# OpenStitching/stitching

Hardware: AMD Instinct MI355X
Metric: warped+blended Mpix/s (higher is better)
Workload: dtype u8/int16 (fixed-point remap, int32 pyramid sums, fp32 weights); 1 GPU; BASELINE config 2: 8 synthetic 4000x3000 frames, one ring; yaw step 38.9 deg = 0.58 hfov (42 % overlap; SURVEY 8(d) names 0.70 hfov); spherical warp + 5-band multiband blend, inputs resident in HBM; frames_per_gpu=8, panoramas_in_flight=2

## Files before the change

include/stitching_amd_debug.h:

```cpp
#ifndef STITCHING_AMD_DEBUG_H
#define STITCHING_AMD_DEBUG_H

#include "stitching_amd.h"

#ifdef __cplusplus
extern "C" {
#endif

int stx_debug_warp_maps(stx_ctx* ctx, int type, float scale, const float K[9], const float R[9], int w, int h, int which,
                        const int rect_xywh[4], stx_buf** out_xmap_f32, stx_buf** out_ymap_f32, int out_xywh[4]);

int stx_debug_feather_dist_cap(void);

int stx_debug_blend_replayed(stx_ctx* ctx, int* out_launches);

int stx_debug_warp_table_launches(stx_ctx* ctx, int* out_launches);

int stx_debug_blend_uploads(stx_ctx* ctx, int* out_uploads);

int stx_debug_blend_mask_stored(stx_ctx* ctx, int* out_stored);

#ifdef __cplusplus
}
#endif
#endif
```

stitching_amd/_lib.py:

```python
import ctypes as C
import os

from .stitching_error import StitchingError

_HERE = os.path.dirname(os.path.abspath(__file__))
LIB_PATH = os.environ.get("STITCHING_AMD_LIB") or os.path.join(_HERE, "libstitching_amd.so")

STX_OK = 0
WARP_PLANE, WARP_AFFINE, WARP_CYLINDRICAL, WARP_SPHERICAL = 0, 1, 2, 3
WARP_TYPE_IDS = {"plane": 0, "affine": 1, "cylindrical": 2, "spherical": 3, "fisheye": 4, "stereographic": 5,
                 "compressedPlaneA2B1": 6, "compressedPlaneA1.5B1": 7, "compressedPlanePortraitA2B1": 8,
                 "compressedPlanePortraitA1.5B1": 9, "paniniA2B1": 10, "paniniA1.5B1": 11, "paniniPortraitA2B1": 12,
                 "paniniPortraitA1.5B1": 13, "mercator": 14, "transverseMercator": 15}
INTER_NEAREST, INTER_LINEAR = 0, 1
BORDER_CONSTANT, BORDER_REFLECT = 0, 2
BLEND_NO, BLEND_FEATHER, BLEND_MULTIBAND = 0, 1, 2
U8, S16, F32 = 0, 1, 2
TRIG_MODES = {"exact": 0, "glibc": 1, "glibc-nofma": 2}
REMAP_MODES = {"q15": 0, "float": 1, "float-fma": 2}
PYRDOWN_MODES = {"scalar": 0, "simd-v": 1, "simd-hv": 3, "simd-v-fma": 5, "simd-hv-fma": 7}
GAIN_MAP_BOUNDED = 1
EXPOSURE_KINDS = {"gain": 1, "gain_blocks": 2, "channel": 3, "channel_blocks": 4}
EXPOSURE_SOLVERS = {"host": 0, "device": 1}
LU_NB, LU_MAX_N = 32, 16384
# ... 79 lines not shown
    "stx_blend_use_weights": [_vp, _vp, _ip],
    "stx_mb_weights_free": [_vp],
    "stx_blend_set_band": [_vp, _i, _i],
    "stx_blend_feed_ex": [_vp, _vp, _vp, _i, _i, _i],
    "stx_blend_contrib_rect": [_vp, _i, _i, _i, _i, _i, _i, _ip, _zp],
    "stx_blend_export_contrib": [_vp, _i, _i, _i, _vpp, _ip],
    "stx_blend_export_contribs": [_vp, _i, _ip, _ip, _ip, _vpp, _ip],
    "stx_blend_build": [_vp],
    "stx_blend_feed_contrib_ex": [_vp, _i, _ip, _vp, _i],
    "stx_buf_flags": [_vp, _ip],
    "stx_strip_rect": [_vp, _i, _i, _i, _i, _i, _i, _ip, _zp],
    "stx_view_rect": [_vp, _i, _i, _i, _i, _i, _i, _i, _i, _ip],
    "stx_strip_pack": [_vp, _vp, _vp, _i, _i, _vpp],
    "stx_strip_pack_batch_ex": [_vp, _i, _vpp, _vpp, _ip, _ip, _i, _vpp],
    "stx_strip_bytes": [_i, _i, _i, _zp],
    "stx_strip_unpack": [_vp, _i, _i, _i, _vpp, _vpp],
    "stx_blend_feed_strips": [_vp, _i, _vpp, _ip, _ip, _ip, _ip, _ip, _i],
    "stx_comm_unique_id": [_ubp],
    "stx_comm_create": [_vp, _i, _i, _ubp, _vpp],
    "stx_comm_exchange_begin_on": [_vp, _vp, _i, _ip, _ip, _vpp, _zp],
    "stx_comm_exchange_end_on": [_vp, _vp],
    "stx_comm_info": [_vp, _ip],
    "stx_comm_destroy": [_vp],
    "stx_prof_enable": [_vp, _i],
    "stx_prof_reset": [_vp],
    "stx_prof_count": [_vp, _ip],
    "stx_prof_get": [_vp, _i, C.c_char_p, _i, C.POINTER(C.c_int64), _dp, _dp],
    "stx_mark": [_vp, _i],
    "stx_mark_elapsed_ms": [_vp, _i, _i, _dp],
    "stx_exposure_stats": [_vp, _i, _i, _vpp, _vpp, _ip, _i, _llp, _ip, _llp, _dp],
    "stx_exposure_solve": [_i, _i, _ip, _dp, _ubp, _dp],
    "stx_set_exposure_solver": [_i],
    "stx_get_exposure_solver": [],
    "stx_exposure_feed_ex": [_vp, _i, _i, _vpp, _vpp, _ip, _i, _i, _i, _dp, _llp, _dp],
    "stx_exposure_solve_device": [_vp, _i, _i, _ip, _dp, _ubp, _dp, _dp],
    "stx_lu_solve_device": [_vp, _i, _dp, _dp, _dp, _dp],
    "stx_seam_find": [_vp, _i, _i, _ip, _ip, _vpp, _vpp, _dp],
    "stx_seam_schedule": [_i, _ip, _ip, _ip, _ip, _ip],
    "stx_color_seam_find": [_vp, _i, _ip, _ip, _vpp, _vpp, _vpp, _dp],
    "stx_crop_lir": [_vp, _vp, _ip, _ip, _dp],
    "stx_features_detect": [_vp, _i, _vpp, _vpp, _i, _i, _i, _ip, _ip, _ip, _ip, C.POINTER(C.c_byte), _ip, _ip, _llp, _ubp, _dp],
    "stx_match_features": [_vp, _i, _vpp, _ip, _vpp, _ip, _i, _i, _i, _d, _u, _ip, _ip, _ubp, _ip, _dp, _dp],
    "stx_match_features_model": [_vp, _i, _vpp, _ip, _vpp, _ip, _i, _i, _i, _d, _u, _i, _ip, _ip, _ubp, _ip, _dp, _dp],
    "stx_ray_problem_create": [_vp, _i, _ip, _llp, _dp, _vpp],
    "stx_ray_problem_eval": [_vp, _i, _dp, _dp, _dp],
    "stx_affine_problem_eval": [_vp, _i, _dp, _dp, _dp],
    "stx_reproj_problem_eval": [_vp, _i, _dp, _dp, _dp],
    "stx_ray_problem_free": [_vp],
    "stx_ingest": [_vp, _i, C.POINTER(ForeignFrame), _i, _i, _vp, _i, _vpp],
    "stx_emit": [_vp, _i, C.POINTER(EmitItem), _i, _i, _vp, _i, _vpp],
    "stx_debug_warp_maps": [_vp, _i, _f, _fp, _fp, _i, _i, _i, _ip, _vpp, _vpp, _ip],
    "stx_debug_feather_dist_cap": [],
    "stx_debug_blend_replayed": [_vp, _ip],
    "stx_debug_warp_table_launches": [_vp, _ip],
    "stx_debug_blend_uploads": [_vp, _ip],
    "stx_debug_blend_mask_stored": [_vp, _ip],
}
EXPORTS = tuple(PROTOTYPES)

_lib = None


def build_hint():
    return "build it with `make -C stitching_amd/csrc` or `python -c 'import __graft_entry__ as g; g.build()'`"


def lib():
    global _lib
    if _lib is not None:
        return _lib
    if not os.path.exists(LIB_PATH):
        raise ImportError(f"{LIB_PATH} is missing: the HIP back end is not built ({build_hint()}). "
                          "stitching_amd has no CPU fallback.")
    L = C.CDLL(LIB_PATH)
    for name, argtypes in PROTOTYPES.items():
        fn = getattr(L, name)
        fn.argtypes = argtypes
        fn.restype = C.c_char_p if name == "stx_last_error" else C.c_int
    _lib = L
    return L


def check(rc):
    if rc != STX_OK:
        msg = lib().stx_last_error()
        raise StitchingError(f"stitching_amd [{rc}]: {msg.decode(errors='replace') if msg else 'unknown error'}")
```

stitching_amd/csrc/stx_blend_fast.hip:

```cpp
#include <algorithm>
#include <cstdlib>

#include "stx_blend_kernels.h"
#include "stx_device_math.h"

using namespace stxd;

namespace {

constexpr int L0_WAVES = 5;
constexpr float WEIGHT_EPS = 1e-5f;
constexpr float INV255 = 0.0039215688593685627f;
constexpr float INV256 = 0.00390625f;

#define STX_GAS __attribute__((address_space(1)))
template <class T> STX_DEV const STX_GAS T* gp(const T* p) { return (const STX_GAS T*)p; }
template <class T> STX_DEV STX_GAS T* gp(T* p) { return (STX_GAS T*)p; }

STX_DEV bool xcd_tile(const StxTileMap& M, uint32_t b, int& tx, int& ty)
{
    if (M.plain) {
        const uint32_t wy = M.tiles_x == 1 ? b : __umulhi(b, M.magic_tx);
        tx = (int)(b - wy * (uint32_t)M.tiles_x);
        ty = (int)wy;
// ... 166 lines not shown
{
    vm0 = vm1 = 0xffffffffu;
    if (__builtin_amdgcn_ballot_w64(lx0 < 0 || lx0 + 8 > iw) != 0ull) {
        const int lo = max(-lx0, 0), hi = min(iw - lx0, 8);
        const uint32_t bits = ((1u << hi) - 1u) & ~((1u << lo) - 1u);
        vm0 = (((bits & 15u) * 0x00204081u) & 0x01010101u) * 0xffu;
        vm1 = (((bits >> 4) * 0x00204081u) & 0x01010101u) * 0xffu;
    }
}
STX_DEV void load_px8_u8(const uint8_t* img0, uint32_t img0_stride, const uint8_t* mask0, uint32_t mask0_stride, int lx0, int ly, uint32_t vm0,
                         uint32_t vm1, uint32_t (&pw)[6], uint32_t (&mw)[2])
{
    const uint32_t off = (uint32_t)ly * img0_stride + (uint32_t)(lx0 * 3 + 64);
    const STX_GAS uint8_t* q = gp(img0) - 64 + (off & ~3u);
    const uint32_t s = off & 3u;
    const v4u d0 = *reinterpret_cast<const STX_GAS v4u_a4*>(q);
    const v4u d1 = *reinterpret_cast<const STX_GAS v4u_a4*>(q + 16);
    pw[0] = __builtin_amdgcn_alignbyte(d0.y, d0.x, s);
    pw[1] = __builtin_amdgcn_alignbyte(d0.z, d0.y, s);
    pw[2] = __builtin_amdgcn_alignbyte(d0.w, d0.z, s);
    pw[3] = __builtin_amdgcn_alignbyte(d1.x, d0.w, s);
    pw[4] = __builtin_amdgcn_alignbyte(d1.y, d1.x, s);
    pw[5] = __builtin_amdgcn_alignbyte(d1.z, d1.y, s);
    const uint32_t moff = (uint32_t)ly * mask0_stride + (uint32_t)(lx0 + 64);
    const STX_GAS uint8_t* mq = gp(mask0) - 64 + (moff & ~3u);
    const uint32_t ms = moff & 3u;
    const uint32_t m0 = *reinterpret_cast<const STX_GAS uint32_t*>(mq), m1 = *reinterpret_cast<const STX_GAS uint32_t*>(mq + 4),
                   m2 = *reinterpret_cast<const STX_GAS uint32_t*>(mq + 8);
    mw[0] = __builtin_amdgcn_alignbyte(m1, m0, ms) & vm0;
    mw[1] = __builtin_amdgcn_alignbyte(m2, m1, ms) & vm1;
}
STX_DEV void load_px8_u8(const StxMbImage& im, int lx0, int ly, uint32_t vm0, uint32_t vm1, uint32_t (&pw)[6], uint32_t (&mw)[2])
{
    load_px8_u8(im.img0, (uint32_t)im.img0_stride, im.mask0, (uint32_t)im.mask0_stride, lx0, ly, vm0, vm1, pw, mw);
}

STX_DEV int s16lo(uint32_t v) { return (int)(short)(v & 0xffffu); }
STX_DEV int s16hi(uint32_t v) { return (int)(short)(v >> 16); }
STX_DEV uint32_t pack16(int lo, int hi) { return ((uint32_t)lo & 0xffffu) | ((uint32_t)hi << 16); }
STX_DEV uint32_t byte_of(const uint32_t* w, int k) { return (w[k >> 2] >> (8 * (k & 3))) & 255u; }

STX_DEV float h5f(float s0, float s1, float s2, float s3, float s4)
{
    return fadd(fadd(fadd(fmul(s2, 6.f), fmul(fadd(s1, s3), 4.f)), s0), s4);
}
STX_DEV int h5i(int s0, int s1, int s2, int s3, int s4) { return s2 * 6 + (s1 + s3) * 4 + s0 + s4; }

constexpr int DN_TOW = 64, DN_TOH = 14, DN_ROWS = 2 * DN_TOH + 3;
constexpr int DN_BAND = 1;
constexpr int LV_WAVES = 1, LV_TH = 2 * LV_WAVES, LV_THREADS = 64 * LV_WAVES;
constexpr int LV_BAND_ROWS = 8;
constexpr int LV_BAND = LV_BAND_ROWS / LV_TH;

STX_DEV void dn_load36(const STX_GAS uint8_t* img, uint32_t off, uint32_t (&w)[9])
{
    const STX_GAS uint8_t* q = img + (off & ~3u);
    const uint32_t s = off & 3u;
    const v4u d0 = *reinterpret_cast<const STX_GAS v4u_a4*>(q);
    const v4u d1 = *reinterpret_cast<const STX_GAS v4u_a4*>(q + 16);
    const v2u d2 = *reinterpret_cast<const STX_GAS v2u_a4*>(q + 32);
    w[0] = __builtin_amdgcn_alignbyte(d0.y, d0.x, s);
    w[1] = __builtin_amdgcn_alignbyte(d0.z, d0.y, s);
    w[2] = __builtin_amdgcn_alignbyte(d0.w, d0.z, s);
    w[3] = __builtin_amdgcn_alignbyte(d1.x, d0.w, s);
    w[4] = __builtin_amdgcn_alignbyte(d1.y, d1.x, s);
    w[5] = __builtin_amdgcn_alignbyte(d1.z, d1.y, s);
    w[6] = __builtin_amdgcn_alignbyte(d1.w, d1.z, s);
    w[7] = __builtin_amdgcn_alignbyte(d2.x, d1.w, s);
    w[8] = __builtin_amdgcn_alignbyte(d2.y, d2.x, s);
}
template <bool MIRROR, int C>
STX_DEV void dn_pack5_channel(const uint32_t* w, short* hs)
{
#define STX_PXB(k) (MIRROR ? 30 - 3 * (k) + C : 3 * (k) + C)
    const pk16 A = pk(pair_u8<STX_PXB(0), STX_PXB(2)>(w)), Bp = pk(pair_u8<STX_PXB(1), STX_PXB(3)>(w));
    const pk16 Cp = pk(pair_u8<STX_PXB(2), STX_PXB(4)>(w)), D = pk(pair_u8<STX_PXB(3), STX_PXB(5)>(w));
    const pk16 E = pk(pair_u8<STX_PXB(4), STX_PXB(6)>(w)), F = pk(pair_u8<STX_PXB(5), STX_PXB(7)>(w));
    const pk16 G = pk(pair_u8<STX_PXB(6), STX_PXB(8)>(w)), H = pk(pair_u8<STX_PXB(7), STX_PXB(9)>(w));
    const pk16 I = pk(pair_u8<STX_PXB(8), STX_PXB(10)>(w));
#undef STX_PXB
    const pk16 o01 = A + E + Cp * pk_splat(6) + (Bp + D) * pk_splat(4);
    const pk16 o23 = E + I + G * pk_splat(6) + (F + H) * pk_splat(4);
    *reinterpret_cast<uint2*>(hs) = make_uint2(unpk(o01), unpk(o23));
}

STX_DEV float4 dn_mask_sums4(const uint32_t (&mb)[3])
{
    const pk16 o01 = pk(pair_u8<0, 2>(mb)) + pk(pair_u8<4, 6>(mb)) + pk(pair_u8<2, 4>(mb)) * pk_splat(6) +
                     (pk(pair_u8<1, 3>(mb)) + pk(pair_u8<3, 5>(mb))) * pk_splat(4);
    const pk16 o23 = pk(pair_u8<4, 6>(mb)) + pk(pair_u8<8, 10>(mb)) + pk(pair_u8<6, 8>(mb)) * pk_splat(6) +
                     (pk(pair_u8<5, 7>(mb)) + pk(pair_u8<7, 9>(mb))) * pk_splat(4);
    return make_float4((float)(unpk(o01) & 0xffffu), (float)(unpk(o01) >> 16), (float)(unpk(o23) & 0xffffu), (float)(unpk(o23) >> 16));
}

struct DnImage0 {
    int fw, fh, iw, ih, left, top;
    uint32_t img0_stride, mask0_stride;
    const uint8_t* img0;
    const uint8_t* mask0;
};
template <bool PK, bool NEAR, bool WEIGHTS, class IM>
STX_DEV void dn_task_level0(const IM& im, int row, int xo, short* hs0, short* hs1, short* hs2, float* hw)
{
    const int by = reflect101_near(row, im.fh) - im.top;
    const bool yin = (unsigned)by < (unsigned)im.ih;
    const int sy = NEAR ? reflect_near(by, im.ih) : reflect(by, im.ih);
    const STX_GAS uint8_t* img = gp(im.img0);
    const uint32_t rowoff = (uint32_t)sy * (uint32_t)im.img0_stride;
    const int c0 = 2 * xo - 2;
    const int a0 = c0 - im.left;
    int px[11][3];
    float f[11];
    if (c0 >= 0 && c0 + 10 < im.fw && a0 >= 0 && a0 + 10 < im.iw) {
        uint32_t w[9];
        dn_load36(img, rowoff + (uint32_t)a0 * 3u, w);
        dn_pack5_channel<false, 0>(w, hs0);
        dn_pack5_channel<false, 1>(w, hs1);
        dn_pack5_channel<false, 2>(w, hs2);
        if (!WEIGHTS) return;
        uint32_t mw[3] = {0u, 0u, 0u};
        if (yin) {
            const uint32_t moff = (uint32_t)by * (uint32_t)im.mask0_stride + (uint32_t)a0;
            const STX_GAS uint8_t* mq = gp(im.mask0) + (moff & ~3u);
            const uint32_t ms = moff & 3u;
            const v4u m = *reinterpret_cast<const STX_GAS v4u_a4*>(mq);
            mw[0] = __builtin_amdgcn_alignbyte(m.y, m.x, ms);
            mw[1] = __builtin_amdgcn_alignbyte(m.z, m.y, ms);
            mw[2] = __builtin_amdgcn_alignbyte(m.w, m.z, ms) & 0x00ffffffu;
        }
        bool packed = PK;
        if (!PK) {
            const uint32_t odd = (mw[0] ^ (((mw[0] >> 7) & 0x01010101u) * 255u)) | (mw[1] ^ (((mw[1] >> 7) & 0x01010101u) * 255u)) |
                                 (mw[2] ^ (((mw[2] >> 7) & 0x01010101u) * 255u));
            packed = __builtin_amdgcn_ballot_w64(odd != 0u) == 0ull;
        }
// ... 435 lines not shown
            for (int j = 0; j < 19; j++) f[j] = wq[reflect101_near(c0 + j, iw)];
        }
        dn_hsum_store_f(f, &s_w[r][4 * q]);
    }
    __syncthreads();
    const int p = tid & 31, rg = tid >> 5;
    const int xo = X0 + 2 * p;
    if (xo >= ow) return;
    const bool two = xo + 1 < ow;
    uint32_t nz = 0u;
#pragma unroll
    for (int rr = 0; rr < 2; rr++) {
        const int yl = 2 * rg + rr, y = Y0 + yl;
        if (yl >= DN_TOH || y >= oh) break;
#pragma unroll
        for (int c = 0; c < 3; c++) {
            int a[5], b[5];
#pragma unroll
            for (int k = 0; k < 5; k++) {
                a[k] = s_h[c][2 * yl + k][p];
                b[k] = s_h[c][2 * yl + k][32 + p];
            }
            const int va = (h5i(a[0], a[1], a[2], a[3], a[4]) + 128) >> 8;
            const int vb = (h5i(b[0], b[1], b[2], b[3], b[4]) + 128) >> 8;
            const uint32_t oo = (uint32_t)c * gopl + (uint32_t)y * gos + (uint32_t)xo;
            if (g8b) {
                STX_GAS uint8_t* o = gp(reinterpret_cast<uint8_t*>(Go_a)) + oo;
                if (two) *reinterpret_cast<STX_GAS uint16_t*>(o) = (uint16_t)((uint32_t)va | ((uint32_t)vb << 8));
                else o[0] = (uint8_t)va;
            } else {
                STX_GAS short* o = gp(reinterpret_cast<short*>(Go_a)) + oo;
                if (two) *reinterpret_cast<STX_GAS uint32_t*>(o) = pack16(va, vb);
                else o[0] = (short)va;
            }
        }
        if (!WEIGHTS) continue;
        float fa[5], fb[5];
#pragma unroll
        for (int k = 0; k < 5; k++) {
            fa[k] = s_w[2 * yl + k][p];
            fb[k] = s_w[2 * yl + k][32 + p];
        }
        const float wa = fmul(h5f(fa[0], fa[1], fa[2], fa[3], fa[4]), INV256);
        const float wb = fmul(h5f(fb[0], fb[1], fb[2], fb[3], fb[4]), INV256);
        STX_GAS float* o = gp(reinterpret_cast<float*>(Wo_a)) + ((uint32_t)y * wost + (uint32_t)xo);
        typedef float v2fl __attribute__((ext_vector_type(2)));
        if (two) { const v2fl wab = {wa, wb}; *reinterpret_cast<STX_GAS v2fl*>(o) = wab; }
        else o[0] = wa;
        nz |= __float_as_uint(wa) | (two ? __float_as_uint(wb) : 0u);
    }
    if (WEIGHTS) dn_note_occ(occ, nz, tid, X0, Y0, ow, oh);
}

STX_DEV int s6(int v) { return (v + 32) >> 6; }

STX_DEV int trunc_small(float v) { return (int)v; }

template <class T>
STX_DEV void up_patch(const T* __restrict__ plane, long long stride, int cw, int ch, int cx, int cy, int up[2][8])
{
    const int rr[3] = {up_idx(cy - 1, ch), cy, up_idx(cy + 1, ch)};
    const bool le = cx == 0, re = cx + 4 >= cw;
    int he[3][4], ho[3][4];
#pragma unroll
    for (int r = 0; r < 3; r++) {
        const T* p = plane + (long long)rr[r] * stride;
        int c[6];
        if (sizeof(T) == 2) {
            const v4u w = *reinterpret_cast<const v4u_a4*>(p + cx - 2);
            c[1] = s16lo(w.y); c[2] = s16hi(w.y); c[3] = s16lo(w.z); c[4] = s16hi(w.z);
            c[0] = s16hi(w.x);
            c[5] = s16lo(w.w);
        } else {
            const v3u w = *reinterpret_cast<const v3u_a4*>(p + cx - 4);
            c[0] = (int)(w.x >> 24);
            c[1] = (int)(w.y & 255u); c[2] = (int)((w.y >> 8) & 255u); c[3] = (int)((w.y >> 16) & 255u); c[4] = (int)(w.y >> 24);
            c[5] = (int)(w.z & 255u);
        }
        if (le) c[0] = c[2];
        if (re) c[5] = c[4];
#pragma unroll
        for (int j = 0; j < 4; j++) {
            he[r][j] = c[j] + 6 * c[j + 1] + c[j + 2];
            ho[r][j] = 4 * (c[j + 1] + c[j + 2]);
        }
    }
#pragma unroll
    for (int j = 0; j < 4; j++) {
        up[0][2 * j] = s6(he[0][j] + 6 * he[1][j] + he[2][j]);
        up[0][2 * j + 1] = s6(ho[0][j] + 6 * ho[1][j] + ho[2][j]);
        up[1][2 * j] = s6(4 * (he[1][j] + he[2][j]));
        up[1][2 * j + 1] = s6(4 * (ho[1][j] + ho[2][j]));
    }
}

template <bool L0, bool MASK_OPT = false>
STX_DEV void level_epilogue(const MbLevelK& P, int X0, int Y0, int (&acc)[2][8][3], float (&ws)[2][8])
{
    int v[2][8][3];
#pragma unroll
    for (int r = 0; r < 2; r++)
#pragma unroll
        for (int j = 0; j < 8; j++) {
            const float den = fadd(ws[r][j], WEIGHT_EPS);
            float q0, q1, q2;
            div3_shared(den, (float)(short)acc[r][j][0], (float)(short)acc[r][j][1], (float)(short)acc[r][j][2], q0, q1, q2);
// ... 1083 lines not shown
#pragma unroll
        for (int c = 0; c < 3; c++) {
            const short* plane = P.up + c * P.up_plane - ((long long)P.up_y0 * P.up_stride + P.up_x0);
            pk16s up[2][4];
            if (!up_patch_pks_math(uw[c], usel, up)) {
                int u32[2][8];
                up_patch(plane, P.up_stride, P.pw >> 1, P.ph >> 1, X0 >> 1, Y0 >> 1, u32);
#pragma unroll
                for (int r = 0; r < 2; r++) {
                    up[r][0] = pks(pack16(u32[r][0], u32[r][2]));
                    up[r][1] = pks(pack16(u32[r][4], u32[r][6]));
                    up[r][2] = pks(pack16(u32[r][1], u32[r][3]));
                    up[r][3] = pks(pack16(u32[r][5], u32[r][7]));
                }
            }
#pragma unroll
            for (int r = 0; r < 2; r++)
#pragma unroll
                for (int q = 0; q < 4; q++) v[r][c][q] = unpks(__builtin_elementwise_add_sat(up[r][q], pks(v[r][c][q])));
        }
    }
#pragma unroll
    for (int r = 0; r < 2; r++) {
        if (Y0 + r >= P.y1) break;
#pragma unroll
        for (int c = 0; c < 3; c++) {
            v4u o;
            o.x = __builtin_amdgcn_perm(v[r][c][2], v[r][c][0], 0x05040100u);
            o.y = __builtin_amdgcn_perm(v[r][c][2], v[r][c][0], 0x07060302u);
            o.z = __builtin_amdgcn_perm(v[r][c][3], v[r][c][1], 0x05040100u);
            o.w = __builtin_amdgcn_perm(v[r][c][3], v[r][c][1], 0x07060302u);
            *reinterpret_cast<STX_GAS v4u*>(gp(P.out) + c * P.out_plane + (long long)(Y0 + r - P.out_y0) * P.out_stride + (X0 - P.out_x0)) = o;
        }
    }
}

static_assert(LV_WAVES == 1, "a cover word is the search of ONE wavefront: a tile of more wavefronts needs a word per wavefront");
__global__ __launch_bounds__(LV_THREADS) void mb_cover_kernel(const StxMbImage* images, int n_images, int level, int x0, int y0, StxTileMap tiles,
                                                              unsigned long long* cover)
{
    const int tid = threadIdx.x;
    int tile_tx, tile_ty;
    if (!xcd_tile(tiles, blockIdx.x, tile_tx, tile_ty)) return;
    const int tile_x = x0 + tile_tx * 512, tile_y = y0 + tile_ty * LV_TH;
    const int Y0 = tile_y + __builtin_amdgcn_readfirstlane(tid >> 6) * 2;
    const bool hit = level == 0 ? mb_tile_hit<true, false>(images, n_images, 0, tile_x, Y0, tid & 63)
                                : mb_tile_hit<false, false>(images, n_images, level, tile_x, Y0, tid & 63);
    const unsigned long long word = __ballot(hit);
    if ((tid & 63) == 0) cover[((Y0 - y0) / LV_TH) * tiles.tiles_x + tile_tx] = word;
}

bool launched_ok() { return hipGetLastError() == hipSuccess; }

}

bool stx_fast_mb_down_batch(stx_ctx* ctx, const StxMbImage* d_images, const StxMbImage* h_images, int n, int level, bool weights)
{
    int mw = 0, mh = 0;
    for (int i = 0; i < n; i++) {
        mw = std::max(mw, (h_images[i].fw >> level) >> 1);
        mh = std::max(mh, (h_images[i].fh >> level) >> 1);
    }
    if (n <= 0 || mw < 1 || mh < 1 || n > 65535) return false;
    StxTileMap M = stx_tile_map((mw + DN_TOW - 1) / DN_TOW, (mh + DN_TOH - 1) / DN_TOH, DN_BAND);
    constexpr int DN_PLAIN_FROM = 3;
    M.plain = level >= DN_PLAIN_FROM;
    bool pk_ok = true;
    for (int i = 0; i < n; i++) pk_ok = pk_ok && !h_images[i].img0_is_s16 && h_images[i].mask_binary;
    dim3 grid(stx_tile_grid(M), 1, n);
    static const unsigned pad_lds = getenv("STITCHING_AMD_D0_LDS") ? (unsigned)atoi(getenv("STITCHING_AMD_D0_LDS")) : 0u;
    if (!weights) {
        if (level == 0 && pk_ok) hipLaunchKernelGGL((mb_down0_lds_kernel<true, false>), grid, dim3(256), pad_lds, ctx->stream, d_images, M);
        else if (level == 0) hipLaunchKernelGGL((mb_down0_lds_kernel<false, false>), grid, dim3(256), 0, ctx->stream, d_images, M);
        else hipLaunchKernelGGL(mb_down_lds_kernel<false>, grid, dim3(256), 0, ctx->stream, d_images, level, M);
    } else if (level == 0 && pk_ok) hipLaunchKernelGGL((mb_down0_lds_kernel<true, true>), grid, dim3(256), pad_lds, ctx->stream, d_images, M);
    else if (level == 0) hipLaunchKernelGGL((mb_down0_lds_kernel<false, true>), grid, dim3(256), 0, ctx->stream, d_images, M);
    else hipLaunchKernelGGL(mb_down_lds_kernel<true>, grid, dim3(256), 0, ctx->stream, d_images, level, M);
    return launched_ok();
}

static bool fast_level_ok(const MbLevelK& K, MbLevelK* KT)
{
    if (K.num_bands - K.level < 3) return false;
    if ((K.x0 | K.y0 | K.out_x0 | K.out_y0 | K.pano_x0 | K.pano_y0) & 7) return false;
    if (K.up && ((K.up_x0 | K.up_y0) & 3)) return false;
    if (K.n_images > 255) return false;
    *KT = K;
    KT->tiles = stx_tile_map((K.x1 - K.x0 + 511) / 512, (K.y1 - K.y0 + LV_TH - 1) / LV_TH, LV_BAND);
    return true;
}

int stx_fast_mb_emit_class(const MbLevelK& K, MbLevelK* KT)
{
    if (!(K.level > 0 || K.all_u8) || !fast_level_ok(K, KT)) { *KT = K; return -1; }
    return K.level == 0 ? 0 : (K.all_u8 ? 1 : 2);
}

bool stx_fast_mb_emit_launch(stx_ctx* ctx, int cls, const MbLevelK* d_Ks, const MbLevelK* h_Ks, int count)
{
    unsigned gx = 1;
    for (int i = 0; i < count; i++) gx = std::max(gx, stx_tile_grid(h_Ks[i].tiles));
    const dim3 grid(gx, 1, (unsigned)count);
    if (cls == 0) hipLaunchKernelGGL((mb_emit_multi_kernel<true, false>), grid, dim3(LV_THREADS), 0, ctx->stream, d_Ks);
    else if (cls == 1) hipLaunchKernelGGL((mb_emit_multi_kernel<false, true>), grid, dim3(LV_THREADS), 0, ctx->stream, d_Ks);
    else hipLaunchKernelGGL((mb_emit_multi_kernel<false, false>), grid, dim3(LV_THREADS), 0, ctx->stream, d_Ks);
    return launched_ok();
}

static bool no_defer()
{
    static const bool off = getenv("STITCHING_AMD_NO_DEFER") != nullptr;
    return off;
}

static bool mb_replays(const MbLevelK& K) { return !K.emit && K.cover != nullptr && K.n_images <= 64 && !K.has_contrib; }
enum MbL0Path { L0_OTHER, L0_PK, L0_DEFER };
// ... 96 lines not shown
```

stitching_amd/csrc/stx_blend_host.cpp:

```cpp
#include <algorithm>
#include <climits>
#include <cmath>
#include <cstdlib>
#include <cstring>
#include <memory>

#include "stx_blend_kernels.h"
#include "stx_internal.h"

STX_EXPORT int stx_debug_feather_dist_cap(void) { return STX_FEATHER_DIST_CAP; }

STX_EXPORT int stx_result_roi(int n, const int* corners_xy, const int* sizes_wh, int out_xywh[4])
{
    if (n <= 0 || !corners_xy || !sizes_wh || !out_xywh) return stx_fail(STX_ERR_INVALID, "bad argument");
    int tlx = INT_MAX, tly = INT_MAX, brx = INT_MIN, bry = INT_MIN;
    for (int i = 0; i < n; i++) {
        tlx = std::min(tlx, corners_xy[2 * i]);
        tly = std::min(tly, corners_xy[2 * i + 1]);
        brx = std::max(brx, corners_xy[2 * i] + sizes_wh[2 * i]);
        bry = std::max(bry, corners_xy[2 * i + 1] + sizes_wh[2 * i + 1]);
    }
    out_xywh[0] = tlx; out_xywh[1] = tly; out_xywh[2] = brx - tlx; out_xywh[3] = bry - tly;
    return STX_OK;
}
// ... 512 lines not shown

STX_EXPORT int stx_blend_keep_weights(stx_blender* b, stx_mb_weights** out)
{
    if (!b || !out) return stx_fail(STX_ERR_INVALID, "null argument");
    *out = nullptr;
    if (b->finished) return stx_fail(STX_ERR_STATE, "keep_weights after blend()");
    if (b->keep) return stx_fail(STX_ERR_STATE, "keep_weights was already called on this blender");
    if (b->images.empty() || !mb_weights_eligible(b, false)) return STX_OK;
    stx_mb_weights* w = new stx_mb_weights();
    w->ctx = b->ctx;
    w->refs = 2;
    b->keep = w;
    *out = w;
    return STX_OK;
}

STX_EXPORT int stx_blend_use_weights(stx_blender* b, stx_mb_weights* w, int* out_adopted)
{
    if (!b || !w || !out_adopted) return stx_fail(STX_ERR_INVALID, "null argument");
    *out_adopted = 0;
    if (b->finished) return stx_fail(STX_ERR_STATE, "use_weights after blend()");
    if (b->ctx != w->ctx) return stx_fail(STX_ERR_INVALID, "use_weights: the handle belongs to another context (no cross-stream use)");
    if (b->adopted || b->keep || w->images.empty() || w->images.size() != b->images.size() || !mb_weights_eligible(b, false)) return STX_OK;
    if (b->num_bands != w->num_bands || b->pyr_mode != w->pyr_mode || b->rx != w->rx || b->ry != w->ry || b->rw != w->rw || b->rh != w->rh)
        return STX_OK;
    for (size_t i = 0; i < b->images.size(); i++) {
        const StxMbImage& im = b->images[i];
        const StxMbKept& k = w->images[i];
        if (b->built[i]) return STX_OK;
        if (im.mask0 != k.mask0 || im.mask0_stride != k.mask0_stride || im.mask_binary != k.mask_binary || im.w1_f16 != k.w1_f16 ||
            im.iw != k.iw || im.ih != k.ih || im.ix != k.ix || im.iy != k.iy || im.fx != k.fx || im.fy != k.fy || im.fw != k.fw ||
            im.fh != k.fh || im.left != k.left || im.top != k.top)
            return STX_OK;
        for (int l = 1; l <= b->num_bands; l++)
            if (im.wt_stride[l] != k.wt_stride[l]) return STX_OK;
    }
    STX_TRY(stx_set_device(b->ctx));
    for (size_t i = 0; i < b->images.size(); i++)
        for (int l = 1; l <= b->num_bands; l++) { b->images[i].wt[l] = w->images[i].wt[l]; b->images[i].occ[l] = w->images[i].occ[l]; }
    b->d_all = nullptr;
    w->refs++;
    b->adopted = w;
    *out_adopted = 1;
    return STX_OK;
}

STX_EXPORT int stx_debug_blend_replayed(stx_ctx* ctx, int* out_launches)
{
    if (!ctx || !out_launches) return stx_fail(STX_ERR_INVALID, "null argument");
    *out_launches = ctx->blend_replayed;
    return STX_OK;
}

STX_EXPORT int stx_debug_blend_mask_stored(stx_ctx* ctx, int* out_stored)
{
    if (!ctx || !out_stored) return stx_fail(STX_ERR_INVALID, "null argument");
    *out_stored = ctx->blend_mask_stored;
    return STX_OK;
}

STX_EXPORT int stx_debug_blend_uploads(stx_ctx* ctx, int* out_uploads)
{
    if (!ctx || !out_uploads) return stx_fail(STX_ERR_INVALID, "null argument");
    *out_uploads = ctx->blend_uploads;
    return STX_OK;
}

STX_EXPORT int stx_mb_weights_free(stx_mb_weights* w)
{
    stx_mb_weights_release(w);
    return STX_OK;
}

STX_EXPORT int stx_blend_set_band(stx_blender* b, int x0, int x1)
{
    if (!b) return stx_fail(STX_ERR_INVALID, "null argument");
    if (b->kind != STX_BLEND_MULTIBAND) return stx_fail(STX_ERR_UNSUPPORTED, "bands exist for the multi-band blender only");
    if (b->finished) return stx_fail(STX_ERR_STATE, "set_band after blend()");
    const int al = (1 << b->num_bands) - 1;
    if (x0 < 0 || x1 > b->fw || x1 <= x0 || (x0 & al) || ((x1 & al) && x1 != b->fw) || (x0 & 7))
        return stx_fail(STX_ERR_INVALID, "band [%d,%d) must lie in [0,%d) with edges on multiples of max(8, 2^bands)", x0, x1, b->fw);
    b->band_x0 = x0; b->band_x1 = x1;
    return STX_OK;
}

STX_EXPORT int stx_blend_contrib_rect(const stx_blender* b, int img_w, int img_h, int tlx, int tly, int band_x0, int band_x1,
                                      int out_rect_xywh[4], size_t* out_bytes)
{
    if (!b || !out_rect_xywh) return stx_fail(STX_ERR_INVALID, "null argument");
    if (b->kind != STX_BLEND_MULTIBAND) return stx_fail(STX_ERR_UNSUPPORTED, "multi-band blender only");
    int fx, fy, fw, fh, sx0, sx1;
    mb_feed_rect(b, img_w, img_h, tlx, tly, &fx, &fy, &fw, &fh);
    if (!mb_contrib_range(b, fx, fw, band_x0, band_x1, &sx0, &sx1)) {
        out_rect_xywh[0] = out_rect_xywh[1] = out_rect_xywh[2] = out_rect_xywh[3] = 0;
        if (out_bytes) *out_bytes = 0;
        return STX_OK;
    }
    out_rect_xywh[0] = sx0; out_rect_xywh[1] = fy; out_rect_xywh[2] = sx1 - sx0; out_rect_xywh[3] = fh;
    if (out_bytes) {
        ContribLayout L;
        mb_contrib_layout(b->num_bands, sx1 - sx0, fh, &L);
        *out_bytes = L.bytes;
    }
    return STX_OK;
}

// ... 123 lines not shown
    b->held.push_back(const_cast<stx_buf*>(packed));
    return STX_OK;
}

static int feather_finish(stx_blender* b, stx_buf* pano, stx_buf* pmask, stx_buf* p16)
{
    stx_ctx* ctx = b->ctx;
    const int n = (int)b->feather_images.size();
    StxDevBlock tab;
    STX_TRY(upload_small(ctx, b->feather_images.data(), sizeof(FeatherImg) * (size_t)n, &tab));
    void* const d_tab = tab.release();
    b->pyr_allocs.push_back(d_tab);
    STX_TRY(stx_launch_feather_weights(ctx, (const FeatherImg*)d_tab, b->feather_images.data(), n));
    double bytes = 4.0 * pano->w * pano->h + (p16 ? 6.0 * pano->w * pano->h : 0.0);
    for (const FeatherImg& im : b->feather_images) bytes += (double)im.w * im.h * ((im.is_s16 ? 6 : 3) + 2);
    FeatherGatherK K;
    K.imgs = (const FeatherImg*)d_tab; K.n = n; K.w = pano->w; K.h = pano->h; K.sharpness = b->sharpness;
    K.pano = pano->ptr; K.pano_stride = (long long)pano->stride; K.pmask = pmask->ptr; K.pmask_stride = (long long)pmask->stride;
    K.pano16 = p16 ? (short*)p16->ptr : nullptr; K.pano16_stride = p16 ? (long long)p16->stride : 0;
    return stx_launch_feather_gather(ctx, K, bytes);
}

static int no_finish(stx_blender* b, stx_buf* pano, stx_buf* pmask, stx_buf* p16)
{
    stx_ctx* ctx = b->ctx;
    const int n = (int)b->no_images.size();
    void* d_tab = nullptr;
    STX_TRY(stx_dev_alloc(ctx, sizeof(NoImg) * std::max(n, 1), &d_tab));
    b->pyr_allocs.push_back(d_tab);
    bool all_binary = true;
    double bytes = 4.0 * pano->w * pano->h + (p16 ? 6.0 * pano->w * pano->h : 0.0);
    for (const NoImg& im : b->no_images) {
        all_binary = all_binary && im.mask_binary;
        bytes += (double)im.w * im.h;
    }
    bytes += 3.0 * pano->w * pano->h;
    if (n > 0) STX_TRY(stx_stage_upload(ctx, d_tab, b->no_images.data(), sizeof(NoImg) * (size_t)n));
    NoGatherK K;
    K.imgs = (const NoImg*)d_tab; K.n = n; K.all_binary = all_binary ? 1 : 0;
    K.w = pano->w; K.h = pano->h;
    K.pano = pano->ptr; K.pano_stride = (long long)pano->stride; K.pmask = pmask->ptr; K.pmask_stride = (long long)pmask->stride;
    K.pano16 = p16 ? (short*)p16->ptr : nullptr; K.pano16_stride = p16 ? (long long)p16->stride : 0;
    return stx_launch_no_gather(ctx, K, bytes);
}

STX_EXPORT int stx_blend_finish_ex(stx_blender* b, stx_buf** out_pano_u8, stx_buf** out_mask_u8, stx_buf** out_pano_s16)
{
    if (!b) return stx_fail(STX_ERR_INVALID, "null argument");
    if (b->finished) return stx_fail(STX_ERR_STATE, "blend() was already called on this blender");
    if (!b->ctx) return stx_fail(STX_ERR_STATE, "geometry-only blender (created without a context)");
    STX_TRY(stx_set_device(b->ctx));
    stx_ctx* ctx = b->ctx;
    ctx->blend_replayed = 0;
    ctx->blend_uploads = 0;
    ctx->blend_mask_stored = 0;
    const int ow = b->kind == STX_BLEND_MULTIBAND ? b->band_x1 - b->band_x0 : b->rw, oh = b->kind == STX_BLEND_MULTIBAND ? b->fh : b->rh;
    StxBufRef p16, pmask, pano;
    const int rc = [&]() {
        STX_TRY(stx_buf_new(ctx, ow, oh, 3, STX_U8, &pano));
        if (b->kind != STX_BLEND_MULTIBAND) STX_TRY(stx_buf_new(ctx, ow, oh, 1, STX_U8, &pmask));
        if (out_pano_s16) STX_TRY(stx_buf_new(ctx, ow, oh, 3, STX_S16, &p16));
        if (b->kind == STX_BLEND_MULTIBAND) return mb_finish(b, pano.get(), &pmask, p16.get());
        if (b->kind == STX_BLEND_NO) return no_finish(b, pano.get(), pmask.get(), p16.get());
        return feather_finish(b, pano.get(), pmask.get(), p16.get());
    }();
    if (rc == STX_OK && b->kind == STX_BLEND_MULTIBAND) mb_hand_over_weights(b, pmask.get());
    b->finished = true;
    blender_release(b);
    STX_TRY(rc);
    if (out_pano_u8) *out_pano_u8 = pano.release();
    if (out_mask_u8) *out_mask_u8 = pmask.release();
    if (out_pano_s16) *out_pano_s16 = p16.release();
    return STX_OK;
}

STX_EXPORT int stx_blend_finish(stx_blender* b, stx_buf** out_pano_u8, stx_buf** out_mask_u8)
{
    return stx_blend_finish_ex(b, out_pano_u8, out_mask_u8, nullptr);
}

STX_EXPORT int stx_blend_destroy(stx_blender* b)
{
    if (!b) return STX_OK;
    if (b->ctx) {
        hipSetDevice(b->ctx->device);
        blender_release(b);
    }
    delete b;
    return STX_OK;
}
```

stitching_amd/csrc/stx_internal.h:

```cpp
#pragma once
#include <hip/hip_runtime.h>

#include <atomic>
#include <cstdarg>
#include <cstddef>
#include <cstdint>
#include <cstdio>
#include <map>
#include <memory>
#include <mutex>
#include <string>
#include <vector>

#include "../../include/stitching_amd.h"
#include "../../include/stitching_amd_debug.h"

#define STX_EXPORT extern "C" __attribute__((visibility("default")))
#define STX_MAX_BANDS 16

void stx_set_error(const char* fmt, ...);
int stx_fail(int code, const char* fmt, ...);

#define STX_HIP(call)                                                                                      \
    do {                                                                                                   \
// ... 3 lines not shown
                            #call, hipGetErrorString(e_), __FILE__, __LINE__);                             \
    } while (0)

inline int stx_check_launch(const char* what)
{
    hipError_t e = hipGetLastError();
    if (e != hipSuccess) return stx_fail(STX_ERR_HIP, "%s launch failed: %s", what, hipGetErrorString(e));
    return STX_OK;
}

#define STX_TRY(call)           \
    do {                        \
        int rc_ = (call);       \
        if (rc_ != STX_OK) return rc_; \
    } while (0)

struct StxProfEntry {
    std::string name;
    int64_t calls = 0;
    double total_ms = 0.0;
    double algo_bytes = 0.0;
};

struct StxPendingEvent {
    hipEvent_t start, stop;
    int entry;
};

struct stx_ctx {
    int device = 0;
    hipStream_t stream = nullptr;
    hipStream_t aux_stream = nullptr;
    void* aux_scratch = nullptr;
    std::mutex alloc_mutex;
    std::map<size_t, std::vector<void*>> free_blocks;
    std::map<void*, size_t> block_size;
    size_t bytes_allocated = 0;
    void* pinned = nullptr;
    size_t pinned_bytes = 0;
    uint32_t roi_seq = 0;
    uint8_t* stage = nullptr;
    size_t stage_bytes = 0, stage_off = 0;
    hipEvent_t stage_ev[4] = {};
    bool stage_ev_set[4] = {};
    int stage_seg = 0;
    bool prof_on = false;
    std::vector<StxProfEntry> prof;
    std::map<std::string, int> prof_index;
    std::vector<StxPendingEvent> prof_pending;
    std::vector<hipEvent_t> event_pool;
    hipEvent_t marks[16] = {};
    double* exp_sqrt = nullptr;
    int blend_replayed = 0;
    int warp_table_launches = 0;
    int blend_uploads = 0;
    int blend_mask_stored = 0;
};

#define STX_STAGE_SEGS 4
int stx_dev_alloc(stx_ctx* ctx, size_t bytes, void** out);
int stx_stage_upload(stx_ctx* ctx, void* d, const void* h, size_t bytes);
void stx_dev_free(stx_ctx* ctx, void* p);
int stx_set_device(stx_ctx* ctx);
struct StxDevFree { stx_ctx* ctx; void operator()(void* p) const { stx_dev_free(ctx, p); } };
using StxDevBlock = std::unique_ptr<void, StxDevFree>;
inline int stx_dev_alloc(stx_ctx* ctx, size_t bytes, StxDevBlock* out)
{
    void* p = nullptr;
    STX_TRY(stx_dev_alloc(ctx, bytes, &p));
    *out = StxDevBlock(p, StxDevFree{ctx});
    return STX_OK;
}
int upload_small(stx_ctx* ctx, const void* h, size_t bytes, StxDevBlock* d_out);
size_t align_up(size_t v, size_t a);

struct StxProfScope {
    stx_ctx* ctx;
    int pending = -1;
    hipStream_t stream;
    bool attached;
    StxProfScope(stx_ctx* c, const char* name, double algo_bytes, hipStream_t on = nullptr, bool attach = false);
    ~StxProfScope();
    hipEvent_t start() const;
    hipEvent_t stop() const;
};

struct stx_buf {
    stx_ctx* ctx = nullptr;
    void* base = nullptr;
    uint8_t* ptr = nullptr;
    int w = 0, h = 0, c = 0, elem = 0;
    size_t stride = 0;
    stx_buf* parent = nullptr;
    int mask_binary = 0;
    std::atomic<int> refs{1};
};

constexpr size_t STX_BUF_FRONT_PAD = 64;
inline int stx_elem_bytes(int elem) { return elem == STX_U8 ? 1 : (elem == STX_S16 ? 2 : 4); }
int stx_buf_new(stx_ctx* ctx, int w, int h, int c, int elem, stx_buf** out);
void stx_buf_retain(stx_buf* b);
void stx_buf_release(stx_buf* b);
struct StxBufRelease { void operator()(stx_buf* b) const { stx_buf_release(b); } };
using StxBufRef = std::unique_ptr<stx_buf, StxBufRelease>;
inline int stx_buf_new(stx_ctx* ctx, int w, int h, int c, int elem, StxBufRef* out)
{
// ... 285 lines not shown
```

Measured before the change: 206,600 Mpix/s.

## Add streaming level-0 pyramid downsample kernel with register-rotated row prefetch

Adds a dedicated kernel for the first multiband pyramid reduction (level 0, no weights). Each 64-thread block covers a 256x16 output tile and streams input rows through four rotating register buffers, issuing loads four rows ahead. The vertical 1-4-6-4-1 filter is kept as running partial sums instead of re-reading a shared tile. A generic coefficient path handles reflected borders, and a byte-wise path handles very narrow images. The goal is to cut shared-memory staging and load latency in the bandwidth-heavy first downsample, at the cost of more code paths and eligibility checks that fall back to the old kernel.

```diff
diff --git a/include/stitching_amd_debug.h b/include/stitching_amd_debug.h
--- a/include/stitching_amd_debug.h
+++ b/include/stitching_amd_debug.h
@@ -14,6 +14,8 @@
 
 int stx_debug_blend_replayed(stx_ctx* ctx, int* out_launches);
 
+int stx_debug_blend_streamed(stx_ctx* ctx, int* out_launches);
+
 int stx_debug_warp_table_launches(stx_ctx* ctx, int* out_launches);
 
 int stx_debug_blend_uploads(stx_ctx* ctx, int* out_uploads);
diff --git a/stitching_amd/_lib.py b/stitching_amd/_lib.py
--- a/stitching_amd/_lib.py
+++ b/stitching_amd/_lib.py
@@ -155,6 +155,7 @@
     "stx_debug_warp_maps": [_vp, _i, _f, _fp, _fp, _i, _i, _i, _ip, _vpp, _vpp, _ip],
     "stx_debug_feather_dist_cap": [],
     "stx_debug_blend_replayed": [_vp, _ip],
+    "stx_debug_blend_streamed": [_vp, _ip],
     "stx_debug_warp_table_launches": [_vp, _ip],
     "stx_debug_blend_uploads": [_vp, _ip],
     "stx_debug_blend_mask_stored": [_vp, _ip],
diff --git a/stitching_amd/csrc/stx_blend_fast.hip b/stitching_amd/csrc/stx_blend_fast.hip
--- a/stitching_amd/csrc/stx_blend_fast.hip
+++ b/stitching_amd/csrc/stx_blend_fast.hip
@@ -242,13 +242,8 @@
 constexpr int LV_BAND_ROWS = 8;
 constexpr int LV_BAND = LV_BAND_ROWS / LV_TH;
 
-STX_DEV void dn_load36(const STX_GAS uint8_t* img, uint32_t off, uint32_t (&w)[9])
-{
-    const STX_GAS uint8_t* q = img + (off & ~3u);
-    const uint32_t s = off & 3u;
-    const v4u d0 = *reinterpret_cast<const STX_GAS v4u_a4*>(q);
-    const v4u d1 = *reinterpret_cast<const STX_GAS v4u_a4*>(q + 16);
-    const v2u d2 = *reinterpret_cast<const STX_GAS v2u_a4*>(q + 32);
+STX_DEV void dn_align36(const v4u d0, const v4u d1, const v2u d2, uint32_t s, uint32_t (&w)[9])
+{
     w[0] = __builtin_amdgcn_alignbyte(d0.y, d0.x, s);
     w[1] = __builtin_amdgcn_alignbyte(d0.z, d0.y, s);
     w[2] = __builtin_amdgcn_alignbyte(d0.w, d0.z, s);
@@ -259,8 +254,16 @@
     w[7] = __builtin_amdgcn_alignbyte(d2.x, d1.w, s);
     w[8] = __builtin_amdgcn_alignbyte(d2.y, d2.x, s);
 }
+STX_DEV void dn_load36(const STX_GAS uint8_t* img, uint32_t off, uint32_t (&w)[9])
+{
+    const STX_GAS uint8_t* q = img + (off & ~3u);
+    const v4u d0 = *reinterpret_cast<const STX_GAS v4u_a4*>(q);
+    const v4u d1 = *reinterpret_cast<const STX_GAS v4u_a4*>(q + 16);
+    const v2u d2 = *reinterpret_cast<const STX_GAS v2u_a4*>(q + 32);
+    dn_align36(d0, d1, d2, off & 3u, w);
+}
 template <bool MIRROR, int C>
-STX_DEV void dn_pack5_channel(const uint32_t* w, short* hs)
+STX_DEV void dn_pack5_pairs(const uint32_t* w, pk16& o01, pk16& o23)
 {
 #define STX_PXB(k) (MIRROR ? 30 - 3 * (k) + C : 3 * (k) + C)
     const pk16 A = pk(pair_u8<STX_PXB(0), STX_PXB(2)>(w)), Bp = pk(pair_u8<STX_PXB(1), STX_PXB(3)>(w));
@@ -269,8 +272,14 @@
     const pk16 G = pk(pair_u8<STX_PXB(6), STX_PXB(8)>(w)), H = pk(pair_u8<STX_PXB(7), STX_PXB(9)>(w));
     const pk16 I = pk(pair_u8<STX_PXB(8), STX_PXB(10)>(w));
 #undef STX_PXB
-    const pk16 o01 = A + E + Cp * pk_splat(6) + (Bp + D) * pk_splat(4);
-    const pk16 o23 = E + I + G * pk_splat(6) + (F + H) * pk_splat(4);
+    o01 = A + E + Cp * pk_splat(6) + (Bp + D) * pk_splat(4);
+    o23 = E + I + G * pk_splat(6) + (F + H) * pk_splat(4);
+}
+template <bool MIRROR, int C>
+STX_DEV void dn_pack5_channel(const uint32_t* w, short* hs)
+{
+    pk16 o01, o23;
+    dn_pack5_pairs<MIRROR, C>(w, o01, o23);
     *reinterpret_cast<uint2*>(hs) = make_uint2(unpk(o01), unpk(o23));
 }
 
@@ -812,6 +821,209 @@
     if (WEIGHTS) dn_note_occ(occ, nz, tid, X0, Y0, ow, oh);
 }
 
+constexpr int DS_COLS = 256, DS_ROWS = 16, DS_BAND = 1;
+struct DsRaw { v4u a, b; v2u c; uint32_t s; };
+struct DsCoef { uint32_t q[11]; };
+struct DsSrc {
+    const STX_GAS uint8_t* src;
+    uint32_t ss;
+    int fw, fh, iw, ih, left, top;
+    int row0, jmax;
+};
+STX_DEV uint32_t ds_rowoff(const DsSrc& K, int j)
+{
+    const int by = reflect101_near(K.row0 + min(j, K.jmax), K.fh) - K.top;
+    return (uint32_t)reflect_near(by, K.ih) * K.ss;
+}
+STX_DEV void ds_issue(const DsSrc& K, int j, uint32_t woff, DsRaw& r)
+{
+    const uint32_t off = ds_rowoff(K, j) + woff;
+    const STX_GAS uint8_t* q = K.src + (off & ~3u);
+    r.s = off & 3u;
+    r.a = *reinterpret_cast<const STX_GAS v4u_a4*>(q);
+    r.b = *reinterpret_cast<const STX_GAS v4u_a4*>(q + 16);
+    r.c = *reinterpret_cast<const STX_GAS v2u_a4*>(q + 32);
+}
+STX_DEV void ds_window(const DsRaw& r, uint32_t (&w)[9]) { dn_align36(r.a, r.b, r.c, r.s, w); }
+STX_DEV void ds_window_bytes(const DsSrc& K, int j, int c0, uint32_t (&w)[9])
+{
+    const uint32_t rowoff = ds_rowoff(K, j);
+#pragma unroll
+    for (int k = 0; k < 9; k++) w[k] = 0u;
+#pragma unroll
+    for (int k = 0; k < 11; k++) {
+        const int sx = reflect_near(reflect101_near(c0 + k, K.fw) - K.left, K.iw);
+#pragma unroll
+        for (int c = 0; c < 3; c++) {
+            const uint32_t v = K.src[rowoff + (uint32_t)sx * 3u + (uint32_t)c];
+            const int pos = 3 * k + c;
+            w[pos >> 2] |= v << (8 * (pos & 3));
+        }
+    }
+}
+STX_DEV void ds_hsum_coef(const uint32_t* w, const DsCoef& Q, pk16 (&h01)[3], pk16 (&h23)[3])
+{
+#pragma unroll
+    for (int c = 0; c < 3; c++) h01[c] = h23[c] = pk_splat(0);
+#pragma unroll
+    for (int s = 0; s < 11; s++) {
+        const pk16 c01 = pk(__builtin_amdgcn_perm(Q.q[s], Q.q[s], 0x0c010c00u)), c23 = pk(__builtin_amdgcn_perm(Q.q[s], Q.q[s], 0x0c030c02u));
+#pragma unroll
+        for (int c = 0; c < 3; c++) {
+            const int k = 3 * s + c;
+            const uint32_t sel = (uint32_t)(k & 3) * 0x00010001u | 0x0c000c00u;
+            const pk16 p = pk(__builtin_amdgcn_perm(w[k >> 2], w[k >> 2], sel));
+            h01[c] += p * c01;
+            h23[c] += p * c23;
+        }
+    }
+}
+STX_DEV void ds_row_sums(const uint32_t (&w)[9], bool generic, const DsCoef& Q, pk16 (&h01)[3], pk16 (&h23)[3])
+{
+    if (generic) {
+        ds_hsum_coef(w, Q, h01, h23);
+    } else {
+        dn_pack5_pairs<false, 0>(w, h01[0], h23[0]);
+        dn_pack5_pairs<false, 1>(w, h01[1], h23[1]);
+        dn_pack5_pairs<false, 2>(w, h01[2], h23[2]);
+    }
+}
+
+template <bool BYTES>
+__global__ __launch_bounds__(64) __attribute__((amdgpu_waves_per_eu(BYTES ? 2 : 4, 8))) void mb_down0_stream_kernel(const StxMbImage* __restrict__ images, StxTileMap M)
+{
+    const uint32_t zz = gridDim.z - 1u - blockIdx.z, bb = gridDim.x - 1u - blockIdx.x;
+    const StxMbImage& im = images[zz];
+    int tile_tx, tile_ty;
+    if (!xcd_tile(M, bb, tile_tx, tile_ty)) return;
+    DsSrc K;
+    uint32_t os, op;
+    unsigned long long oa;
+    {
+        int fw = im.fw, fh = im.fh, iw = im.iw, ih = im.ih, left = im.left, top = im.top;
+        uint32_t ss = (uint32_t)im.img0_stride;
+        unsigned long long sa = (unsigned long long)im.img0;
+        os = (uint32_t)im.g_stride[1]; op = (uint32_t)im.g_plane[1];
+        oa = (unsigned long long)im.g[1];
+        asm volatile("" : "+s"(fw), "+s"(fh), "+s"(iw), "+s"(ih), "+s"(left), "+s"(top), "+s"(ss), "+s"(sa), "+s"(os), "+s"(op), "+s"(oa));
+        K.src = gp(reinterpret_cast<const uint8_t*>(sa));
+        K.ss = ss; K.fw = fw; K.fh = fh; K.iw = iw; K.ih = ih; K.left = left; K.top = top;
+    }
+    const int ow = K.fw >> 1, oh = K.fh >> 1;
+    const int X0 = tile_tx * DS_COLS, Y0 = tile_ty * DS_ROWS;
+    if (X0 >= ow || Y0 >= oh) return;
+    const int n = min(DS_ROWS, oh - Y0);
+    K.row0 = 2 * Y0 - 2;
+    K.jmax = 2 * n + 2;
+    const int xo = X0 + 4 * (int)threadIdx.x;
+    const int c0 = 2 * min(xo, (ow - 1) & ~3) - 2;
+    const bool bytes = BYTES && K.iw < 11;
+    int rel[11];
+    uint32_t woff;
+    {
+        int sx[11], smin = 0x7fffffff;
+#pragma unroll
+        for (int k = 0; k < 11; k++) {
+            sx[k] = reflect_near(reflect101_near(c0 + k, K.fw) - K.left, K.iw);
+            smin = min(smin, sx[k]);
+        }
+        const int wstart = bytes ? 0 : min(smin, K.iw - 11);
+#pragma unroll
+        for (int k = 0; k < 11; k++) rel[k] = bytes ? k : min(sx[k] - wstart, 10);
+        woff = (uint32_t)wstart * 3u;
+    }
+    bool in_order = true;
+#pragma unroll
+    for (int k = 0; k < 11; k++) in_order = in_order && rel[k] == k;
+    const bool generic = __builtin_amdgcn_ballot_w64(!in_order) != 0ull;
+    DsCoef Q;
+#pragma unroll
+    for (int s = 0; s < 11; s++) Q.q[s] = 0u;
+    if (generic) {
+        unsigned long long acc[4] = {0ull, 0ull, 0ull, 0ull};
+#pragma unroll
+        for (int o = 0; o < 4; o++) {
+            acc[o] += 1ull << (5 * rel[2 * o]);
+            acc[o] += 4ull << (5 * rel[2 * o + 1]);
+            acc[o] += 6ull << (5 * rel[2 * o + 2]);
+            acc[o] += 4ull << (5 * rel[2 * o + 3]);
+            acc[o] += 1ull << (5 * rel[2 * o + 4]);
+        }
+#pragma unroll
+        for (int s = 0; s < 11; s++) {
+            Q.q[s] = ((uint32_t)(acc[0] >> (5 * s)) & 31u) | (((uint32_t)(acc[1] >> (5 * s)) & 31u) << 8) |
+                     (((uint32_t)(acc[2] >> (5 * s)) & 31u) << 16) | (((uint32_t)(acc[3] >> (5 * s)) & 31u) << 24);
+        }
+    }
+    STX_GAS uint8_t* const dst = gp(reinterpret_cast<uint8_t*>(oa));
+    const int live = min(ow - xo, 4);
+
+    DsRaw r0, r1, r2, r3;
+    if (!bytes) {
+        ds_issue(K, 0, woff, r0);
+        ds_issue(K, 1, woff, r1);
+        ds_issue(K, 2, woff, r2);
+        ds_issue(K, 3, woff, r3);
+    }
+    __builtin_amdgcn_sched_barrier(0);
+    pk16 P01[3], P23[3], N01[3], N23[3];
+#define STX_DS_ROW(r, j, h01, h23)                                   \
+    {                                                                \
+        uint32_t w[9];                                               \
+        if (bytes) ds_window_bytes(K, (j), c0, w);               \
+        else {                                                       \
+            ds_window(r, w);                                           \
+            ds_issue(K, (j) + 4, woff, r);                       \
+        }                                                            \
+        __builtin_amdgcn_sched_barrier(0);                           \
+        ds_row_sums(w, generic, Q, h01, h23);                    \
+    }
+#define STX_DS_STEP(ro, re, i)                                                                                  \
+    {                                                                                                           \
+        pk16 h01[3], h23[3];                                                                                    \
+        STX_DS_ROW(ro, 2 * (i) + 1, h01, h23)                                                                   \
+        _Pragma("unroll") for (int c = 0; c < 3; c++) {                                                         \
+            P01[c] += h01[c] * pk_splat(4); P23[c] += h23[c] * pk_splat(4);                                     \
+            N01[c] += h01[c] * pk_splat(4); N23[c] += h23[c] * pk_splat(4);                                     \
+        }                                                                                                       \
+        STX_DS_ROW(re, 2 * (i) + 2, h01, h23)                                                                   \
+        const int y = Y0 + (i) - 1;                                                                             \
+        _Pragma("unroll") for (int c = 0; c < 3; c++) {                                                         \
+            const pk16 v01 = (P01[c] + h01[c] + pk_splat(128)) >> pk_splat(8);                                  \
+            const pk16 v23 = (P23[c] + h23[c] + pk_splat(128)) >> pk_splat(8);                                  \
+            P01[c] = N01[c] + h01[c] * pk_splat(6); P23[c] = N23[c] + h23[c] * pk_splat(6);                     \
+            N01[c] = h01[c]; N23[c] = h23[c];                                                                   \
+            if ((i) >= 1 && live > 0) {                                                                         \
+                const uint32_t b4 = __builtin_amdgcn_perm(unpk(v23), unpk(v01), 0x06040200u);                   \
+                STX_GAS uint8_t* o = dst + ((uint32_t)c * op + (uint32_t)y * os + (uint32_t)xo);                \
+                if (live == 4) *reinterpret_cast<STX_GAS uint32_t*>(o) = b4;                                    \
+                else {                                                                                          \
+                    o[0] = (uint8_t)b4;                                                                         \
+                    if (live > 1) o[1] = (uint8_t)(b4 >> 8);                                                    \
+                    if (live > 2) o[2] = (uint8_t)(b4 >> 16);                                                   \
+                }                                                                                               \
+            }                                                                                                   \
+        }                                                                                                       \
+    }
+    {
+        pk16 h01[3], h23[3];
+        STX_DS_ROW(r0, 0, h01, h23)
+#pragma unroll
+        for (int c = 0; c < 3; c++) {
+            P01[c] = P23[c] = pk_splat(0);
+            N01[c] = h01[c]; N23[c] = h23[c];
+        }
+    }
+    int i = 0;
+    for (; i < n; i += 2) {
+        STX_DS_STEP(r1, r2, i)
+        STX_DS_STEP(r3, r0, i + 1)
+    }
+    if (i == n) STX_DS_STEP(r1, r2, i)
+#undef STX_DS_STEP
+#undef STX_DS_ROW
+}
+
 STX_DEV int s6(int v) { return (v + 32) >> 6; }
 
 STX_DEV int trunc_small(float v) { return (int)v; }
@@ -2001,6 +2213,20 @@
 
 bool launched_ok() { return hipGetLastError() == hipSuccess; }
 
+bool mb_down_streams(const StxMbImage* h_images, int n, int level, bool weights)
+{
+    if (weights || level != 0) return false;
+    for (int i = 0; i < n; i++) {
+        const StxMbImage& im = h_images[i];
+        if (im.kind != 0 || !im.g_u8) return false;
+        if (!(im.left >= 0 && im.top >= 0 && im.left <= im.iw && im.fw - im.left - im.iw <= im.iw && im.top <= im.ih && im.fh - im.top - im.ih <= im.ih)) return false;
+        if (im.img0_stride <= 0 || im.img0_stride >= (1ll << 24) || im.g_stride[1] <= 0 || im.g_stride[1] >= (1ll << 24)) return false;
+        if ((long long)im.ih * im.img0_stride + 64 >= (1ll << 32) || 3 * im.g_plane[1] >= (1ll << 32)) return false;
+        if ((im.g_stride[1] | im.g_plane[1]) & 3) return false;
+    }
+    return true;
+}
+
 }
 
 bool stx_fast_mb_down_batch(stx_ctx* ctx, const StxMbImage* d_images, const StxMbImage* h_images, int n, int level, bool weights)
@@ -2011,6 +2237,16 @@
         mh = std::max(mh, (h_images[i].fh >> level) >> 1);
     }
     if (n <= 0 || mw < 1 || mh < 1 || n > 65535) return false;
+    if (mb_down_streams(h_images, n, level, weights)) {
+        const StxTileMap S = stx_tile_map((mw + DS_COLS - 1) / DS_COLS, (mh + DS_ROWS - 1) / DS_ROWS, DS_BAND);
+        const dim3 sgrid(stx_tile_grid(S), 1, n);
+        bool narrow = false;
+        for (int i = 0; i < n; i++) narrow = narrow || h_images[i].iw < 11;
+        if (narrow) hipLaunchKernelGGL(mb_down0_stream_kernel<true>, sgrid, dim3(64), 0, ctx->stream, d_images, S);
+        else hipLaunchKernelGGL(mb_down0_stream_kernel<false>, sgrid, dim3(64), 0, ctx->stream, d_images, S);
+        ctx->blend_streamed++;
+        return launched_ok();
+    }
     StxTileMap M = stx_tile_map((mw + DN_TOW - 1) / DN_TOW, (mh + DN_TOH - 1) / DN_TOH, DN_BAND);
     constexpr int DN_PLAIN_FROM = 3;
     M.plain = level >= DN_PLAIN_FROM;
diff --git a/stitching_amd/csrc/stx_blend_host.cpp b/stitching_amd/csrc/stx_blend_host.cpp
--- a/stitching_amd/csrc/stx_blend_host.cpp
+++ b/stitching_amd/csrc/stx_blend_host.cpp
@@ -588,6 +588,13 @@
     return STX_OK;
 }
 
+STX_EXPORT int stx_debug_blend_streamed(stx_ctx* ctx, int* out_launches)
+{
+    if (!ctx || !out_launches) return stx_fail(STX_ERR_INVALID, "null argument");
+    *out_launches = ctx->blend_streamed;
+    return STX_OK;
+}
+
 STX_EXPORT int stx_debug_blend_mask_stored(stx_ctx* ctx, int* out_stored)
 {
     if (!ctx || !out_stored) return stx_fail(STX_ERR_INVALID, "null argument");
@@ -817,6 +824,7 @@
     STX_TRY(stx_set_device(b->ctx));
     stx_ctx* ctx = b->ctx;
     ctx->blend_replayed = 0;
+    ctx->blend_streamed = 0;
     ctx->blend_uploads = 0;
     ctx->blend_mask_stored = 0;
     const int ow = b->kind == STX_BLEND_MULTIBAND ? b->band_x1 - b->band_x0 : b->rw, oh = b->kind == STX_BLEND_MULTIBAND ? b->fh : b->rh;
diff --git a/stitching_amd/csrc/stx_internal.h b/stitching_amd/csrc/stx_internal.h
--- a/stitching_amd/csrc/stx_internal.h
+++ b/stitching_amd/csrc/stx_internal.h
@@ -79,6 +79,7 @@
     hipEvent_t marks[16] = {};
     double* exp_sqrt = nullptr;
     int blend_replayed = 0;
+    int blend_streamed = 0;
     int warp_table_launches = 0;
     int blend_uploads = 0;
     int blend_mask_stored = 0;
```

New measurement: 209,700 Mpix/s (median of 6 runs). About the same (+1.5%).
